# heyblackC/DFMIR

Hardware: AMD Instinct MI355X
Metric: train-step image-pairs/sec (fwd+bwd): 2D 256x256 bs=16 and 3D 160^3 bs=1 (higher is better)
Workload: dtype f32 (fp16x2-split MFMA, fp32 accumulate)

## Files before the change

dfmir_amd/_lib.py:

```python
import ctypes
import os
from ctypes import c_float, c_int, c_longlong, c_void_p, POINTER, Structure

_HERE = os.path.dirname(os.path.abspath(__file__))
LIB_PATH = os.environ.get("DFMIR_HIP_LIB") or os.path.join(_HERE, "libdfmir_hip.so")


class DfConvGeom(Structure):
    _fields_ = [(n, c_int) for n in (
        "N", "Cin", "Cout", "Di", "Hi", "Wi", "Do", "Ho", "Wo", "KD", "KH", "KW",
        "stride", "dil", "pd", "ph", "pw", "pad_mode", "act")] + [("slope", c_float)]


P = c_void_p
_GP = POINTER(DfConvGeom)
_SIGS = {
    "dfmir_abi_version": [],
    "dfmir_set_option": [ctypes.c_char_p, ctypes.c_char_p],
    "dfmir_get_option": [ctypes.c_char_p, ctypes.c_char_p, c_int],
    "dfmir_conv_fwd": [_GP, P, P, P, P, P],
    "dfmir_conv_wgrad": [_GP, P, P, P, P],
    "dfmir_bias_grad": [P, P, c_int, c_int, c_longlong, P],
    "dfmir_weight_pack": [P, P, c_int, c_int, c_int, c_int, P],
    "dfmir_weight_pack_floats": [c_int, c_int, c_int],
# ... 93 lines not shown
    "dfmir_patch_gather_bwd_amax": [P, P, P, c_int, c_int, c_longlong, c_int, P, P],
    "dfmir_patch_gather_fwd_g": [P, P, P, c_int, c_int, c_longlong, c_int, c_int, P],
    "dfmir_patch_gather_bwd_g": [P, P, P, c_int, c_int, c_longlong, c_int, c_int, P, P],
    "dfmir_l2norm_fwd": [P, P, P, c_int, c_longlong, c_float, P],
    "dfmir_l2norm_bwd": [P, P, P, P, c_int, c_longlong, c_float, P],
    "dfmir_patchnce_fwd": [P, P, P, P, c_longlong, c_int, c_int, c_float, P],
    "dfmir_patchnce_bwd": [P, P, P, P, c_longlong, c_int, c_int, c_float, P],
    "dfmir_masked_l1_fwd": [P, P, P, c_float, P, P, c_longlong, P],
    "dfmir_masked_l1_bwd": [P, P, P, c_float, P, P, P, P, c_longlong, P],
    "dfmir_flow_smooth_ws_floats": [],
    "dfmir_flow_smooth_fwd": [P, P, P] + [c_int] * 5 + [P],
    "dfmir_flow_smooth_bwd": [P, P, P] + [c_int] * 5 + [P],
    "dfmir_flow_smooth_fwd_p": [P, P, P] + [c_int] * 6 + [P],
    "dfmir_flow_smooth_bwd_p": [P, P, P] + [c_int] * 6 + [P],
    "dfmir_mul": [P, P, P, c_longlong, P],
    "dfmir_nmi_ws_floats": [c_longlong, c_int],
    "dfmir_nmi_fwd": [P, P, P, P, c_int, c_float, c_float, c_longlong, P, P, P],
    "dfmir_nmi_bwd": [P, P, P, P, c_int, c_float, c_float, c_longlong, P, P, P, P, P],
    "dfmir_warp_dice_ws_floats": [c_int] * 6,
    "dfmir_warp_dice_fwd": [c_int, P, P, P, P] + [c_int] * 6 + [P, P, P, P, P],
    "dfmir_warp_dice_bwd": [c_int, P, P, P, P] + [c_int] * 5 + [P, P, P, P],
    "dfmir_dice_ws_floats": [c_longlong, c_longlong],
    "dfmir_dice_fwd": [P, P, c_longlong, c_longlong, P, P, P],
    "dfmir_dice_bwd": [P, P, c_longlong, c_longlong, P, P, P, P, P],
    "dfmir_mse_ws_floats": [c_longlong],
    "dfmir_mse_fwd": [P, P, c_longlong, P, P, P],
    "dfmir_mse_bwd": [P, P, c_longlong, P, P, P, P],
    "dfmir_ncc_fwd_m": [P, P, P, c_int, P, P, P, P] + [c_int] * 5 + [c_float, P],
    "dfmir_ncc_bwd_m": [P, P, P, c_int, P, P, P, P, P, P] + [c_int] * 5 + [c_float, P],
    "dfmir_ncc_fwd": [P, P, P, P, P, P] + [c_int] * 5 + [c_float, P],
    "dfmir_ncc_bwd": [P, P, P, P, P, P, P, P] + [c_int] * 5 + [c_float, P],
    "dfmir_patch_gather_fwd_multi": [P, c_int, P, P, c_int, c_int, c_longlong, c_int, P],
    "dfmir_nce_head_fwd": [P, c_int, P, P, P, P, P, P, P, P, P, P, c_int, c_int, c_longlong, c_int, c_float, P],
    "dfmir_patch_ids_draw": [P, P, c_int, c_int, c_int, P, P],
    "dfmir_segment_means_fwd": [P, P, c_int, c_int, c_longlong, c_float, P],
    "dfmir_segment_means_bwd": [P, P, c_int, c_int, c_longlong, c_float, P],
    "dfmir_scalar_combine_fwd": [P, c_int, P, c_int, P, P],
    "dfmir_scalar_combine_bwd": [P, c_int, P, c_int, P, P],
    "dfmir_det_head_floats": [],
    "dfmir_det_begin": [P, c_longlong, P, c_longlong, P, c_int, P, c_longlong, P, c_int, ctypes.c_double, P],
    "dfmir_det_end": [P, P, c_longlong, P, c_longlong, P],
    "dfmir_fill_zero": [P, c_longlong, P],
    "dfmir_sum_scaled": [P, P, c_longlong, c_float, P],
    "dfmir_fill_from_scalar": [P, P, c_longlong, c_float, P],
    "dfmir_adam_step": [P, P, P, P, c_longlong] + [c_float] * 7 + [P],
}

_lib = None


class DfmirHipError(RuntimeError):
    pass


def lib():
    global _lib
    if _lib is None:
        import torch
        if not os.path.exists(LIB_PATH):
            raise DfmirHipError(
                "libdfmir_hip.so not found at %s -- build it with `python -c 'import __graft_entry__ as g; "
                "g.build()'` or `make -C dfmir_amd/csrc` (there is no CPU fallback)" % LIB_PATH)
        h = ctypes.CDLL(LIB_PATH)
        for name, args in _SIGS.items():
            fn = getattr(h, name)
            fn.argtypes = args
# ... 38 lines not shown
```

dfmir_amd/csrc/nce_head.hip:

```cpp
#include "common.h"

#define DF_IDS_MAXP 1024
#define DF_IDS_MAXPERM 4096
struct DfIdSizes {
  long long S[8];
};

__device__ __forceinline__ unsigned long long df_mix64(unsigned long long z) {
  z += 0x9E3779B97F4A7C15ull;
  z = (z ^ (z >> 30)) * 0xBF58476D1CE4E5B9ull;
  z = (z ^ (z >> 27)) * 0x94D049BB133111EBull;
  return z ^ (z >> 31);
}

__global__ __launch_bounds__(256) void patch_ids_draw_k(unsigned long long* __restrict__ state, DfIdSizes sizes,
                                                        int n_layers, int n_sets, int P, int Ppad,
                                                        long long* __restrict__ out) {
  __shared__ unsigned long long el[DF_IDS_MAXPERM];
  __shared__ unsigned char lost[DF_IDS_MAXP];
  __shared__ int pending;
  const int layer = blockIdx.x / n_sets, set = blockIdx.x - layer * n_sets;
  const unsigned long long S = (unsigned long long)sizes.S[layer];
  const unsigned long long seed = state[0], counter = state[1];
  const unsigned long long stream = df_mix64(seed ^ df_mix64(counter * 0x100000001B3ull + (unsigned long long)blockIdx.x));
// ... 253 lines not shown
  __syncthreads();
  const float nr = sqrtf((red[0][l31] + red[1][l31]) + (red[2][l31] + red[3][l31]));
  const float inv = 1.f / (nr + k.eps);
  const long long rr = r0 + l31;
  if (rr < k.rows) {
    if (k.nrm && wid == 0 && hi == 0) k.nrm[rr] = nr;
#pragma unroll
    for (int i = 0; i < 2; ++i)
#pragma unroll
      for (int e = 0; e < 16; ++e) {
        const int m = m0 + 32 * i + (e >> 2) * 8 + hi * 4 + (e & 3);
        k.out[(long long)m * k.rows + rr] = acc[i][e] * inv;
        if (k.ypre) k.ypre[(long long)m * k.rows + rr] = acc[i][e];
      }
  }
}
extern "C" int dfmir_nce_head_fwd(const float* const* srcs, int G, const long long* ids, const float* w1, const float* b1,
                                  const float* w2, const float* b2, float* out, float* nrm, float* xs, float* hs,
                                  float* ypre, int Bper, int C, long long S, int P, float eps, void* stream) {
  DF_ARG_CHECK(srcs && ids && w1 && b1 && w2 && b2 && out && G > 0 && G <= 8 && Bper > 0 && C > 0 && C <= NH_CMAX && S > 0 && P > 0);
  NceHeadP k{};
  for (int g = 0; g < G; ++g) {
    DF_ARG_CHECK(srcs[g] != nullptr);
    k.srcs.p[g] = srcs[g];
  }
  k.ids = ids; k.w1 = w1; k.b1 = b1; k.w2 = w2; k.b2 = b2;
  k.out = out; k.nrm = nrm; k.xs = xs; k.hs = hs; k.ypre = ypre;
  k.G = G; k.Bper = Bper; k.C = C; k.P = P; k.S = S; k.rows = (long long)G * Bper * P; k.eps = eps;
  nce_head_fwd_k<<<(unsigned)((k.rows + NH_R - 1) / NH_R), 256, 0, (hipStream_t)stream>>>(k);
  DF_LAUNCH_CHECK();
  return 0;
}

__global__ __launch_bounds__(256) void segment_means_k(const float* __restrict__ rows, float* __restrict__ out, int L,
                                                       int T, long long seg, float scale) {
  __shared__ float sm[17];
  const int t = blockIdx.x;
  float s = 0.f;
  for (int l = 0; l < L; ++l) {
    const float* r = rows + ((long long)l * T + t) * seg;
    for (long long i = threadIdx.x; i < seg; i += 256) s += r[i];
  }
  s = block_sum(s, sm);
  if (threadIdx.x == 0) out[t] = s * (scale / (float)seg);
}
__global__ void segment_means_bwd_k(const float* __restrict__ g, float* __restrict__ drows, int L, int T, long long seg,
                                    float scale) {
  const long long total = (long long)L * T * seg;
  for (long long i = (long long)blockIdx.x * blockDim.x + threadIdx.x; i < total;
       i += (long long)gridDim.x * blockDim.x) {
    const int t = (int)((i / seg) % T);
    drows[i] = g[t] * (scale / (float)seg);
  }
}
extern "C" int dfmir_segment_means_fwd(const float* rows, float* out, int L, int T, long long seg, float scale,
                                       void* stream) {
  DF_ARG_CHECK(rows && out && L > 0 && T > 0 && seg > 0);
  segment_means_k<<<(unsigned)T, 256, 0, (hipStream_t)stream>>>(rows, out, L, T, seg, scale);
  DF_LAUNCH_CHECK();
  return 0;
}
extern "C" int dfmir_segment_means_bwd(const float* gout, float* drows, int L, int T, long long seg, float scale,
                                       void* stream) {
  DF_ARG_CHECK(gout && drows && L > 0 && T > 0 && seg > 0);
  segment_means_bwd_k<<<df_grid((long long)L * T * seg, 256, 1024), 256, 0, (hipStream_t)stream>>>(gout, drows, L, T, seg,
                                                                                                scale);
// ... 60 lines not shown
```

dfmir_amd/csrc/patchnce.hip:

```cpp
#include "common.h"

__global__ void patch_gather_fwd_k(const float* __restrict__ feat, const long long* __restrict__ ids,
                                   float* __restrict__ out, int B, int C, long long S, int P, int bpg) {
  const long long total = (long long)B * C * P;
  for (long long i = (long long)blockIdx.x * blockDim.x + threadIdx.x; i < total;
       i += (long long)gridDim.x * blockDim.x) {
    const int p = (int)(i % P);
    const long long bc = i / P;
    const long long b = bc / C, c = bc - b * C;
    out[c * ((long long)B * P) + b * P + p] = feat[bc * S + ids[(b / bpg) * P + p]];
  }
}
template <bool DISTINCT>
__global__ void patch_gather_bwd_k(const float* __restrict__ dout, const long long* __restrict__ ids,
                                   float* __restrict__ dfeat, int B, int C, long long S, int P, int bpg,
                                   unsigned* __restrict__ amax, unsigned* __restrict__ pmax = nullptr) {
  const long long total = (long long)B * C * P;
  for (long long i = (long long)blockIdx.x * blockDim.x + threadIdx.x; i < total;
       i += (long long)gridDim.x * blockDim.x) {
    int p;
    long long bc, b, c;
    if (total < 0x7FFFFFFFLL) {
      const unsigned u = (unsigned)i;
      p = (int)(u % (unsigned)P);
      const unsigned ubc = u / (unsigned)P;
      bc = ubc; b = ubc / (unsigned)C; c = ubc - (unsigned)b * (unsigned)C;
    } else {
      p = (int)(i % P);
      bc = i / P;
      b = bc / C; c = bc - b * C;
    }
    const float v = dout[c * ((long long)B * P) + b * P + p];
    float* dst = &dfeat[bc * S + ids[(b / bpg) * P + p]];
    float old;
    if (DISTINCT) { old = *dst; *dst = old + v; }
    else old = atomicAdd(dst, v);
    if (amax) {
      float nv = fabsf(old + v);
      if (!(nv == nv)) nv = __uint_as_float(0x7f800000u);
      unsigned* sl = amax + (bc & (DF_PROBE_SLOTS - 1));
      if (__float_as_uint(nv) > *reinterpret_cast<volatile unsigned*>(sl)) atomicMax(sl, __float_as_uint(nv));
      if (pmax && __float_as_uint(nv) > *reinterpret_cast<volatile unsigned*>(pmax + bc)) atomicMax(pmax + bc, __float_as_uint(nv));
    }
  }
}

__global__ __launch_bounds__(256) void l2norm_fwd_k(const float* __restrict__ x, float* __restrict__ y,
                                                    float* __restrict__ nrm, int C, long long P, float eps) {
  __shared__ float red[16][17];
  const int r = threadIdx.x & 15, cg = threadIdx.x >> 4;
  const long long i = (long long)blockIdx.x * 16 + r;
  const bool ok = i < P;
  float s = 0.f;
  if (ok)
    for (int c = cg; c < C; c += 16) {
      const float v = x[(long long)c * P + i];
      s += v * v;
    }
  red[cg][r] = s;
  __syncthreads();
  float tot = 0.f;
#pragma unroll
  for (int g = 0; g < 16; ++g) tot += red[g][r];
  if (!ok) return;
  const float n = sqrtf(tot);
  if (cg == 0) nrm[i] = n;
  const float inv = 1.f / (n + eps);
  for (int c = cg; c < C; c += 16) y[(long long)c * P + i] = x[(long long)c * P + i] * inv;
}
__global__ __launch_bounds__(256) void l2norm_bwd_k(const float* __restrict__ dy, const float* __restrict__ x,
                                                    const float* __restrict__ nrm, float* __restrict__ dx, int C,
                                                    long long P, float eps) {
  __shared__ float red[16][17];
  const int r = threadIdx.x & 15, cg = threadIdx.x >> 4;
  const long long i = (long long)blockIdx.x * 16 + r;
  const bool ok = i < P;
  float s = 0.f;
  if (ok)
    for (int c = cg; c < C; c += 16) s += dy[(long long)c * P + i] * x[(long long)c * P + i];
// ... 286 lines not shown
  const long long r = r0 + l15;
  const float dpos = (probs[r * ld] - 1.f) * dloss[r] * invT;
#pragma unroll
  for (int t = 0; t < 4; ++t) {
    const int ct = wid * 4 + t;
    if (ct >= ntile) continue;
#pragma unroll
    for (int e = 0; e < 4; ++e) {
      const long long off = (long long)(ct * 16 + lk * 4 + e) * rows + r;
      dq[off] = acc[t][e] + dpos * k[off];
    }
  }
}

extern "C" int dfmir_patch_gather_fwd(const float* feat, const long long* ids, float* out, int B, int C,
                                      long long S, int P, void* stream) {
  DF_ARG_CHECK(feat && ids && out && B > 0 && C > 0 && S > 0 && P > 0);
  patch_gather_fwd_k<<<df_grid((long long)B * C * P, 256, 4096), 256, 0, (hipStream_t)stream>>>(
      feat, ids, out, B, C, S, P, B);
  DF_LAUNCH_CHECK();
  return 0;
}
extern "C" int dfmir_patch_gather_fwd_g(const float* feat, const long long* ids, float* out, int B, int C,
                                        long long S, int P, int G, void* stream) {
  DF_ARG_CHECK(feat && ids && out && B > 0 && C > 0 && S > 0 && P > 0 && G > 0 && B % G == 0);
  patch_gather_fwd_k<<<df_grid((long long)B * C * P, 256, 4096), 256, 0, (hipStream_t)stream>>>(
      feat, ids, out, B, C, S, P, B / G);
  DF_LAUNCH_CHECK();
  return 0;
}
extern "C" int dfmir_patch_gather_bwd_g(const float* dout, const long long* ids, float* dfeat, int B, int C,
                                        long long S, int P, int G, float* dfeat_amax, void* stream) {
  DF_ARG_CHECK(dout && ids && dfeat && B > 0 && C > 0 && S > 0 && P > 0 && G > 0 && B % G == 0);
  patch_gather_bwd_k<true><<<df_grid((long long)B * C * P, 256, 4096), 256, 0, (hipStream_t)stream>>>(
      dout, ids, dfeat, B, C, S, P, B / G, reinterpret_cast<unsigned*>(dfeat_amax));
  DF_LAUNCH_CHECK();
  return 0;
}
extern "C" int dfmir_patch_gather_bwd_gp(const float* dout, const long long* ids, float* dfeat, int B, int C,
                                         long long S, int P, int G, float* dfeat_amax, float* dfeat_pmax, void* stream) {
  DF_ARG_CHECK(dout && ids && dfeat && dfeat_amax && dfeat_pmax && B > 0 && C > 0 && S > 0 && P > 0 && G > 0 && B % G == 0);
  patch_gather_bwd_k<true><<<df_grid((long long)B * C * P, 256, 4096), 256, 0, (hipStream_t)stream>>>(
      dout, ids, dfeat, B, C, S, P, B / G, reinterpret_cast<unsigned*>(dfeat_amax), reinterpret_cast<unsigned*>(dfeat_pmax));
  DF_LAUNCH_CHECK();
  return 0;
}
extern "C" int dfmir_patch_gather_bwd_any(const float* dout, const long long* ids, float* dfeat, int B, int C,
                                          long long S, int P, int G, float* dfeat_amax, float* dfeat_pmax, void* stream) {
  DF_ARG_CHECK(dout && ids && dfeat && B > 0 && C > 0 && S > 0 && P > 0 && G > 0 && B % G == 0);
  DF_ARG_CHECK(dfeat_amax || !dfeat_pmax);
  patch_gather_bwd_k<false><<<df_grid((long long)B * C * P, 256, 4096), 256, 0, (hipStream_t)stream>>>(
      dout, ids, dfeat, B, C, S, P, B / G, reinterpret_cast<unsigned*>(dfeat_amax), reinterpret_cast<unsigned*>(dfeat_pmax));
  DF_LAUNCH_CHECK();
  return 0;
}
extern "C" int dfmir_patch_gather_bwd(const float* dout, const long long* ids, float* dfeat, int B, int C,
                                      long long S, int P, void* stream) {
  DF_ARG_CHECK(dout && ids && dfeat && B > 0 && C > 0 && S > 0 && P > 0);
  patch_gather_bwd_k<false><<<df_grid((long long)B * C * P, 256, 4096), 256, 0, (hipStream_t)stream>>>(
      dout, ids, dfeat, B, C, S, P, B, nullptr);
  DF_LAUNCH_CHECK();
  return 0;
}
extern "C" int dfmir_patch_gather_bwd_amax(const float* dout, const long long* ids, float* dfeat, int B, int C,
                                           long long S, int P, float* dfeat_amax, void* stream) {
  DF_ARG_CHECK(dout && ids && dfeat && dfeat_amax && B > 0 && C > 0 && S > 0 && P > 0);
  patch_gather_bwd_k<true><<<df_grid((long long)B * C * P, 256, 4096), 256, 0, (hipStream_t)stream>>>(
      dout, ids, dfeat, B, C, S, P, B, reinterpret_cast<unsigned*>(dfeat_amax));
  DF_LAUNCH_CHECK();
  return 0;
}
extern "C" int dfmir_l2norm_fwd(const float* x, float* y, float* norm, int C, long long rows, float eps,
                                void* stream) {
  DF_ARG_CHECK(x && y && norm && C > 0 && rows > 0);
  l2norm_fwd_k<<<(unsigned)((rows + 15) / 16), 256, 0, (hipStream_t)stream>>>(x, y, norm, C, rows, eps);
  DF_LAUNCH_CHECK();
  return 0;
}
extern "C" int dfmir_l2norm_bwd(const float* dy, const float* x, const float* norm, float* dx, int C,
                                long long rows, float eps, void* stream) {
  DF_ARG_CHECK(dy && x && norm && dx && C > 0 && rows > 0);
  l2norm_bwd_k<<<(unsigned)((rows + 15) / 16), 256, 0, (hipStream_t)stream>>>(dy, x, norm, dx, C, rows, eps);
  DF_LAUNCH_CHECK();
  return 0;
}
extern "C" int dfmir_patchnce_fwd(const float* q, const float* k, float* loss, float* probs, long long rows,
                                  int C, int G, float T, void* stream) {
  DF_ARG_CHECK(q && k && loss && probs && rows > 0 && C > 0 && G > 0 && T > 0.f);
  DF_ARG_CHECK(rows % G == 0);
  const int R = (int)(rows / G);
  DF_ARG_CHECK(R % NCE_TI == 0);
  if (R == 256 && C <= 256 && (C & 31) == 0) {
    patchnce_fwd_mfma_k<<<(unsigned)(rows / NCE_TI), 256, 0, (hipStream_t)stream>>>(q, k, loss, probs, rows, C, 1.f / T);
    DF_LAUNCH_CHECK();
    return 0;
  }
  const size_t sh = ((size_t)C * NCE_TI + 32 + 3 * NCE_TI) * sizeof(float);
  DF_ARG_CHECK(sh <= 64 * 1024);
  patchnce_fwd_k<<<(unsigned)(rows / NCE_TI), 256, sh, (hipStream_t)stream>>>(q, k, loss, probs, rows, C, R,
                                                                         1.f / T);
  DF_LAUNCH_CHECK();
// ... 21 lines not shown
```

dfmir_amd/ops.py:

```python
import ctypes
import os

import torch
from torch.autograd import Function
from torch.autograd.function import once_differentiable

from ._lib import DfConvGeom, DfmirHipError, check, lib

_VP = ctypes.c_void_p


def _p(t):
    return None if t is None else _VP(t.data_ptr())


def _st():
    return _VP(torch.cuda.current_stream().cuda_stream)


def _need(*ts):
    for t in ts:
        if t is None:
            continue
        if not t.is_cuda:
# ... 1859 lines not shown
def draw_patch_ids(sizes, n_sets, P, device):
    device = _cuda_device(device)
    st = _IDS_STATE.get(device)
    if st is None:
        st = seed_patch_ids(torch.initial_seed(), device)
    L = len(sizes)
    out = torch.empty((L, n_sets, P), device=device, dtype=torch.int64)
    sz = (ctypes.c_longlong * L)(*[int(s) for s in sizes])
    check(lib().dfmir_patch_ids_draw(_p(st), sz, L, int(n_sets), int(P), _p(out), _st()))
    return mark_distinct(out)


def patch_gather_multi(srcs, ids):
    _need(*srcs)
    _need(ids)
    G = len(srcs)
    srcs = [_c(s) for s in srcs]
    Bper, C = srcs[0].shape[0], srcs[0].shape[1]
    S = srcs[0].numel() // (Bper * C)
    for s_ in srcs:
        if tuple(s_.shape) != tuple(srcs[0].shape):
            raise DfmirHipError("patch_gather_multi: sources differ in shape")
    ids = _c(ids.to(torch.int64))
    if ids.dim() != 2 or ids.shape[0] != G:
        raise DfmirHipError("patch_gather_multi: ids must be [G, P]")
    Pn = ids.shape[1]
    out = torch.empty((C, G * Bper * Pn), device=srcs[0].device, dtype=torch.float32)
    ptrs = (ctypes.c_void_p * G)(*[s_.data_ptr() for s_ in srcs])
    check(lib().dfmir_patch_gather_fwd_multi(ptrs, G, _p(ids), _p(out), Bper, C, S, Pn, _st()))
    return out


_NO_NCE_FUSED = _env_on("DFMIR_NO_NCE_FUSED")


def nce_head_ok(C, nc, use_mlp):
    return use_mlp and not _NO_NCE_FUSED and nc == 256 and 1 <= C <= 256


def _nce_head_launch(ptrs, G, ids, mlp0, mlp2, Bper, C, S, Pn, eps, device, save):
    rows = G * Bper * Pn
    out = torch.empty((256, rows), device=device, dtype=torch.float32)
    nrm = xs = hs = ypre = None
    if save:
        nrm = torch.empty(rows, device=device, dtype=torch.float32)
        xs = torch.empty((C, rows), device=device, dtype=torch.float32)
        hs = torch.empty((256, rows), device=device, dtype=torch.float32)
        ypre = torch.empty((256, rows), device=device, dtype=torch.float32)
    arr = (ctypes.c_void_p * G)(*ptrs)
    check(lib().dfmir_nce_head_fwd(arr, G, _p(ids), _p(mlp0.packed(0)), _p(mlp0.bias), _p(mlp2.packed(0)), _p(mlp2.bias),
                                   _p(out), _p(nrm), _p(xs), _p(hs), _p(ypre), Bper, C, S, Pn, float(eps), _st()))
    return out, nrm, xs, hs, ypre


def nce_head_multi(srcs, ids, mlp0, mlp2, eps=1e-7):
    _need(*srcs)
    srcs = [_c(s_) for s_ in srcs]
    Bper, C = srcs[0].shape[0], srcs[0].shape[1]
    S = srcs[0].numel() // (Bper * C)
    ids = _c(ids.to(torch.int64))
    out, _, _, _, _ = _nce_head_launch([s_.data_ptr() for s_ in srcs], len(srcs), ids, mlp0, mlp2, Bper, C, S, ids.shape[1], eps,
                                       srcs[0].device, False)
    return out


class NceHeadFn(Function):

    @staticmethod
    def forward(ctx, feat, ids, w1, b1, w2, b2, mlp0, mlp2, eps, distinct):
        _need(feat, ids)
        ctx.stash = getattr(feat, "_df_tap_stash", None) if feat.is_contiguous() else None
        feat = _c(feat)
        ids = _c(ids.to(torch.int64))
        G, Pn = ids.shape
        B, C = feat.shape[0], feat.shape[1]
        if B % G:
            raise DfmirHipError("nce_head: ids [G,P] with G dividing the batch")
        Bper = B // G
        S = feat.numel() // (B * C)
        base = feat.data_ptr()
        ptrs = [base + 4 * g * Bper * C * S for g in range(G)]
        out, nrm, xs, hs, ypre = _nce_head_launch(ptrs, G, ids, mlp0, mlp2, Bper, C, S, Pn, eps, feat.device, True)
        ctx.save_for_backward(ids, nrm, xs, hs, ypre, w1, w2)
        ctx.meta = (tuple(feat.shape), B, C, S, Pn, G, bool(distinct), float(eps))
        ctx.mods = (mlp0, mlp2)
        return out

    @staticmethod
    @once_differentiable
    def backward(ctx, dout):
        ids, nrm, xs, hs, ypre, w1, w2 = ctx.saved_tensors
        shape, B, C, S, Pn, G, distinct, eps = ctx.meta
        mlp0, mlp2 = ctx.mods
        rows = B * Pn
        dout = _c(dout)
        dy = torch.empty_like(ypre)
        check(lib().dfmir_l2norm_bwd(_p(dout), _p(ypre), _p(nrm), _p(dy), 256, rows, eps, _st()))
        c2 = _Ctx()
        c2.cfg, c2.x_amax, c2.dead_tail, c2.in_act, c2.has_bias = (2, (1, 1, 1), 1, (0, 0, 0), 0, 0, 0.0, mlp2), None, 0, None, True
        c2.needs_input_grad = (True, ctx.needs_input_grad[4], ctx.needs_input_grad[5])
        dh, dw2, db2 = _conv_backward_impl(c2, dy.view(1, 256, 1, rows), None, hs.view(1, 256, 1, 1, rows),
                                           w2.view(256, 256, 1, 1), None)
        c1 = _Ctx()
        c1.cfg, c1.x_amax, c1.dead_tail, c1.in_act, c1.has_bias = (2, (1, 1, 1), 1, (0, 0, 0), 0, 1, 0.0, mlp0), None, 0, None, True
        c1.needs_input_grad = (ctx.needs_input_grad[0], ctx.needs_input_grad[2], ctx.needs_input_grad[3])
        dx, dw1, db1 = _conv_backward_impl(c1, dh, None, xs.view(1, C, 1, 1, rows), w1.view(256, C, 1, 1),
                                           hs.view(1, 256, 1, 1, rows))
        dfeat = None
        if dx is not None:
            dxr = _c(dx).view(C, rows)
            meta = (shape, B, C, S, Pn, G, distinct)
            if ctx.stash is not None:
                ctx.stash.append((dxr, ids, meta))
            else:
                dfeat = zeros(shape, dxr.device)
                if distinct:
                    check(lib().dfmir_patch_gather_bwd_g(_p(dxr), _p(ids), _p(dfeat), B, C, S, Pn, G, None, _st()))
                else:
                    check(lib().dfmir_patch_gather_bwd_any(_p(dxr), _p(ids), _p(dfeat), B, C, S, Pn, G, None, None, _st()))
        dw1 = dw1.view(256, C) if dw1 is not None else None
        dw2 = dw2.view(256, 256) if dw2 is not None else None
        return dfeat, None, dw1, db1, dw2, db2, None, None, None, None


def nce_head(feat, ids, mlp0, mlp2, eps=1e-7):
    groups = ids.shape[0] if ids.dim() == 2 else 1
    ids2 = ids if ids.dim() == 2 else ids.view(1, -1)
    distinct = ids_distinct(ids, groups) if (torch.is_grad_enabled() and feat.requires_grad) else True
    return NceHeadFn.apply(feat, ids2, mlp0.weight, mlp0.bias, mlp2.weight, mlp2.bias, mlp0, mlp2, eps, distinct)


_LAST_L1_WS = [None]


class MaskedL1Fn(Function):
    @staticmethod
    def forward(ctx, a, b, mask, thr):
        _need(a, b, mask)
        a, b = _c(a), _c(b)
        m = None
# ... 441 lines not shown
```

include/dfmir_hip.h:

```cpp
#ifndef DFMIR_HIP_H
#define DFMIR_HIP_H

#ifdef __cplusplus
extern "C" {
#endif

#define DFMIR_ABI_VERSION 14

int dfmir_abi_version(void);
const char* dfmir_last_error(void);

int dfmir_set_option(const char* name, const char* value);
int dfmir_get_option(const char* name, char* buf, int buf_len);

typedef struct DfConvGeom {
  int N, Cin, Cout;
  int Di, Hi, Wi;
  int Do, Ho, Wo;
  int KD, KH, KW;
  int stride, dil;
  int pd, ph, pw;
  int pad_mode;
  int act;
  float slope;
// ... 169 lines not shown
                     float* dflow, int B, int C, int D, int H, int W, int add_identity,
                     int flow_into_src, void* stream);
long long dfmir_warp_bwd_own_ws_floats(int nd, int B, int C, int D, int H, int W);
int dfmir_warp_bwd_own(int nd, const float* dout, const float* src, const float* flow, float* dsrc, float* dflow, int B,
                       int C, int D, int H, int W, int add_identity, int flow_into_src, float* ws, void* stream);

int dfmir_resize_fwd(const float* x, float* y, int planes, int Di, int Hi, int Wi, int Do, int Ho,
                     int Wo, float mult, void* stream);
int dfmir_resize_bwd(const float* dy, float* dx, int planes, int Di, int Hi, int Wi, int Do, int Ho,
                     int Wo, float mult, void* stream);
long long dfmir_resize_bwd_ws_floats(int planes, int Di, int Hi, int Wi, int Do, int Ho, int Wo);
int dfmir_resize_bwd_sep(const float* dy, float* dx, int planes, int Di, int Hi, int Wi, int Do, int Ho, int Wo,
                         float mult, float* ws, void* stream);

int dfmir_patch_gather_fwd(const float* feat, const long long* ids, float* out, int B, int C,
                           long long S, int P, void* stream);
int dfmir_patch_gather_bwd(const float* dout, const long long* ids, float* dfeat, int B, int C,
                           long long S, int P, void* stream);
int dfmir_patch_gather_bwd_amax(const float* dout, const long long* ids, float* dfeat, int B, int C, long long S,
                                int P, float* dfeat_amax, void* stream);
int dfmir_patch_gather_fwd_g(const float* feat, const long long* ids, float* out, int B, int C, long long S, int P,
                             int G, void* stream);
int dfmir_patch_gather_bwd_g(const float* dout, const long long* ids, float* dfeat, int B, int C, long long S, int P,
                             int G, float* dfeat_amax, void* stream);
int dfmir_patch_gather_bwd_gp(const float* dout, const long long* ids, float* dfeat, int B, int C, long long S, int P,
                              int G, float* dfeat_amax, float* dfeat_pmax, void* stream);
int dfmir_patch_gather_bwd_any(const float* dout, const long long* ids, float* dfeat, int B, int C, long long S, int P,
                               int G, float* dfeat_amax, float* dfeat_pmax, void* stream);
int dfmir_patch_gather_fwd_multi(const float* const* srcs, int G, const long long* ids, float* out, int Bper, int C,
                                 long long S, int P, void* stream);
int dfmir_nce_head_fwd(const float* const* srcs, int G, const long long* ids, const float* w1, const float* b1,
                       const float* w2, const float* b2, float* out, float* nrm, float* xs, float* hs, float* ypre,
                       int Bper, int C, long long S, int P, float eps, void* stream);
int dfmir_patch_ids_draw(unsigned long long* state, const long long* sizes, int n_layers, int n_sets, int P,
                         long long* out, void* stream);
int dfmir_l2norm_fwd(const float* x, float* y, float* norm, int C, long long rows, float eps, void* stream);
int dfmir_l2norm_bwd(const float* dy, const float* x, const float* norm, float* dx, int C,
                     long long rows, float eps, void* stream);
int dfmir_patchnce_fwd(const float* q, const float* k, float* loss, float* probs, long long rows,
                       int C, int G, float T, void* stream);
int dfmir_patchnce_bwd(const float* dloss, const float* probs, const float* k, float* dq,
                       long long rows, int C, int G, float T, void* stream);

int dfmir_masked_l1_fwd(const float* a, const float* b, const unsigned char* mask, float thr,
                        float* ws, float* out, long long n, void* stream);
int dfmir_masked_l1_bwd(const float* a, const float* b, const unsigned char* mask, float thr,
                        const float* ws, const float* gout, float* da, float* db, long long n,
                        void* stream);
long long dfmir_flow_smooth_ws_floats(void);
int dfmir_flow_smooth_fwd(const float* flow, float* ws, float* out, int B, int C, int D, int H,
                          int W, void* stream);
int dfmir_flow_smooth_bwd(const float* flow, const float* gout, float* dflow, int B, int C, int D,
                          int H, int W, void* stream);
int dfmir_flow_smooth_fwd_p(const float* flow, float* ws, float* out, int B, int C, int D, int H,
                            int W, int penalty, void* stream);
int dfmir_flow_smooth_bwd_p(const float* flow, const float* gout, float* dflow, int B, int C, int D,
                            int H, int W, int penalty, void* stream);
long long dfmir_nmi_ws_floats(long long n, int nb);
int dfmir_nmi_fwd(const float* y_true, const float* y_pred, const float* mask, const float* centers, int nb,
                  float preterm, float max_clip, long long n, float* ws, float* out, void* stream);
int dfmir_nmi_bwd(const float* y_true, const float* y_pred, const float* mask, const float* centers, int nb,
                  float preterm, float max_clip, long long n, const float* ws, const float* gout, float* d_true,
                  float* d_pred, void* stream);
long long dfmir_warp_dice_ws_floats(int nd, int B, int K, int D, int H, int W);
int dfmir_warp_dice_fwd(int nd, const unsigned char* mov, const unsigned char* fix, const float* flow,
                        const unsigned char* slot_of, int K, int B, int D, int H, int W, int mode, float* ws,
// ... 46 lines not shown
```

Measured before the change: 216.2.

## Fuse PatchNCE MLP head backward into data and weight-gradient kernels

Replaces the generic path for the PatchNCE projection-head backward (l2norm backward plus two 1x1 conv backwards) with two dedicated kernels. One fuses the l2norm backward, the w2 data-gradient GEMM, the ReLU mask and the w1 data-gradient GEMM per row tile using MFMA. The other computes both weight and bias gradients in a single launch with atomics. It also adds a wave-cooperative patch-gather backward scatter that reduces the amax/pmax atomics to one per wave per group. The new path uses plain fp32 MFMA instead of the split path and atomic accumulation, so summation order and numerics can differ; the old path stays behind an env flag and deterministic mode.

```diff
diff --git a/dfmir_amd/_lib.py b/dfmir_amd/_lib.py
--- a/dfmir_amd/_lib.py
+++ b/dfmir_amd/_lib.py
@@ -149,6 +149,8 @@
     "dfmir_ncc_bwd": [P, P, P, P, P, P, P, P] + [c_int] * 5 + [c_float, P],
     "dfmir_patch_gather_fwd_multi": [P, c_int, P, P, c_int, c_int, c_longlong, c_int, P],
     "dfmir_nce_head_fwd": [P, c_int, P, P, P, P, P, P, P, P, P, P, c_int, c_int, c_longlong, c_int, c_float, P],
+    "dfmir_nce_head_bwd_data": [P, P, P, P, P, P, P, P, P, c_int, c_longlong, c_float, P],
+    "dfmir_nce_head_bwd_wgrad": [P, P, P, P, P, P, P, P, c_int, c_longlong, P],
     "dfmir_patch_ids_draw": [P, P, c_int, c_int, c_int, P, P],
     "dfmir_segment_means_fwd": [P, P, c_int, c_int, c_longlong, c_float, P],
     "dfmir_segment_means_bwd": [P, P, c_int, c_int, c_longlong, c_float, P],
diff --git a/dfmir_amd/csrc/nce_head.hip b/dfmir_amd/csrc/nce_head.hip
--- a/dfmir_amd/csrc/nce_head.hip
+++ b/dfmir_amd/csrc/nce_head.hip
@@ -309,6 +309,243 @@
   return 0;
 }
 
+struct NceHeadBwdP {
+  const float *dout, *ypre, *nrm, *hs, *w1, *w2;
+  float *dy, *dh, *dx;
+  int C;
+  long long rows;
+  float eps;
+};
+__global__ __launch_bounds__(256, 2) void nce_head_bwd_data_k(NceHeadBwdP k) {
+  __shared__ float DYs[NH_M * NH_R];
+  __shared__ float DHs[NH_M * NH_R];
+  __shared__ float red[8][NH_R];
+  const int tid = threadIdx.x, lane = tid & 63, wid = tid >> 6;
+  const int l31 = lane & 31, hi = lane >> 5;
+  const long long r0 = (long long)blockIdx.x * NH_R;
+  {
+    const int r = tid & 31, cg = tid >> 5;
+    const long long rr = r0 + r;
+    const bool rok = rr < k.rows;
+    float s = 0.f;
+#pragma unroll 8
+    for (int m = cg; m < NH_M; m += 8) {
+      const float g = rok ? k.dout[(long long)m * k.rows + rr] : 0.f;
+      const float y = rok ? k.ypre[(long long)m * k.rows + rr] : 0.f;
+      DYs[m * NH_R + r] = g;
+      DHs[m * NH_R + r] = y;
+      s += g * y;
+    }
+    red[cg][r] = s;
+    __syncthreads();
+    float dot = 0.f;
+#pragma unroll
+    for (int g = 0; g < 8; ++g) dot += red[g][r];
+    const float n = rok ? k.nrm[rr] : 0.f;
+    const float inv = 1.f / (n + k.eps);
+    const float k2 = n > 0.f ? dot * inv * inv / n : 0.f;
+#pragma unroll 8
+    for (int m = cg; m < NH_M; m += 8) {
+      const float v = DYs[m * NH_R + r] * inv - DHs[m * NH_R + r] * k2;
+      DYs[m * NH_R + r] = v;
+      if (rok) k.dy[(long long)m * k.rows + rr] = v;
+    }
+  }
+  __syncthreads();
+  const int m0 = 64 * wid;
+  const long long rr = r0 + l31;
+  const bool rok = rr < k.rows;
+  nh_f32x16 acc[2];
+#pragma unroll
+  for (int i = 0; i < 2; ++i)
+#pragma unroll
+    for (int e = 0; e < 16; ++e) acc[i][e] = 0.f;
+#define NHB_GEMM(W_, LD_, MB_, SRC_)                                                              \
+  {                                                                                               \
+    const bool ok0 = m0 + l31 < (MB_), ok1 = m0 + l31 + 32 < (MB_);                               \
+    const float* wp = (W_) + m0 + l31;                                                            \
+    constexpr int nb = NH_M / 2 / NH_KB;                                                          \
+    float ca0[NH_KB], ca1[NH_KB], na0[NH_KB], na1[NH_KB];                                         \
+    _Pragma("unroll") for (int u = 0; u < NH_KB; ++u) {                                           \
+      const int kr = 2 * u + hi;                                                                  \
+      ca0[u] = ok0 ? wp[(long long)kr * (LD_)] : 0.f;                                             \
+      ca1[u] = ok1 ? wp[(long long)kr * (LD_) + 32] : 0.f;                                        \
+    }                                                                                             \
+    for (int j = 0; j < nb; ++j) {                                                                \
+      if (j + 1 < nb) {                                                                           \
+        _Pragma("unroll") for (int u = 0; u < NH_KB; ++u) {                                       \
+          const int kr = 2 * ((j + 1) * NH_KB + u) + hi;                                          \
+          na0[u] = ok0 ? wp[(long long)kr * (LD_)] : 0.f;                                         \
+          na1[u] = ok1 ? wp[(long long)kr * (LD_) + 32] : 0.f;                                    \
+        }                                                                                         \
+      }                                                                                           \
+      _Pragma("unroll") for (int u = 0; u < NH_KB; ++u) {                                         \
+        const int kr = 2 * (j * NH_KB + u) + hi;                                                  \
+        const float bv = (SRC_)[kr * NH_R + l31];                                                 \
+        acc[0] = __builtin_amdgcn_mfma_f32_32x32x2f32(ca0[u], bv, acc[0], 0, 0, 0);               \
+        acc[1] = __builtin_amdgcn_mfma_f32_32x32x2f32(ca1[u], bv, acc[1], 0, 0, 0);               \
+      }                                                                                           \
+      _Pragma("unroll") for (int u = 0; u < NH_KB; ++u) { ca0[u] = na0[u]; ca1[u] = na1[u]; }     \
+    }                                                                                             \
+  }
+  float hv[2][16];
+#pragma unroll
+  for (int i = 0; i < 2; ++i)
+#pragma unroll
+    for (int e = 0; e < 16; ++e) {
+      const int m = m0 + 32 * i + (e >> 2) * 8 + hi * 4 + (e & 3);
+      hv[i][e] = rok ? k.hs[(long long)m * k.rows + rr] : 0.f;
+    }
+  NHB_GEMM(k.w2, NH_M, NH_M, DYs)
+#pragma unroll
+  for (int i = 0; i < 2; ++i)
+#pragma unroll
+    for (int e = 0; e < 16; ++e) {
+      const int m = m0 + 32 * i + (e >> 2) * 8 + hi * 4 + (e & 3);
+      const float v = hv[i][e] > 0.f ? acc[i][e] : acc[i][e] * 0.f;
+      DHs[m * NH_R + l31] = v;
+      if (rok) k.dh[(long long)m * k.rows + rr] = v;
+      acc[i][e] = 0.f;
+    }
+  if (!k.dx) return;
+  __syncthreads();
+  if (m0 >= k.C) return;
+  NHB_GEMM(k.w1, k.C, k.C, DHs)
+#undef NHB_GEMM
+  if (rok) {
+#pragma unroll
+    for (int i = 0; i < 2; ++i)
+#pragma unroll
+      for (int e = 0; e < 16; ++e) {
+        const int c = m0 + 32 * i + (e >> 2) * 8 + hi * 4 + (e & 3);
+        if (c < k.C) k.dx[(long long)c * k.rows + rr] = acc[i][e];
+      }
+  }
+}
+extern "C" int dfmir_nce_head_bwd_data(const float* dout, const float* ypre, const float* nrm, const float* hs,
+                                       const float* w1, const float* w2, float* dy, float* dh, float* dx, int C,
+                                       long long rows, float eps, void* stream) {
+  DF_ARG_CHECK(dout && ypre && nrm && hs && w2 && dy && dh && (w1 || !dx) && C > 0 && C <= NH_CMAX && rows > 0 &&
+               rows < (1LL << 31) * NH_R);
+  NceHeadBwdP k{};
+  k.dout = dout; k.ypre = ypre; k.nrm = nrm; k.hs = hs; k.w1 = w1; k.w2 = w2;
+  k.dy = dy; k.dh = dh; k.dx = dx; k.C = C; k.rows = rows; k.eps = eps;
+  nce_head_bwd_data_k<<<(unsigned)((rows + NH_R - 1) / NH_R), 256, 0, (hipStream_t)stream>>>(k);
+  DF_LAUNCH_CHECK();
+  return 0;
+}
+
+struct NceHeadWgP {
+  const float *xs, *hs, *dy, *dh;
+  float *dw1, *db1, *dw2, *db2;
+  int C, nt2;
+  long long rows, chunks, cpb;
+};
+__global__ __launch_bounds__(256) void nce_head_bwd_wgrad_k(NceHeadWgP k) {
+  constexpr int BK = 64, LD = BK + 1;
+  __shared__ float Xs[64 * LD];
+  __shared__ float Ds[64 * LD];
+  const int tid = threadIdx.x, lane = tid & 63, wid = tid >> 6;
+  const int l31 = lane & 31, lhi = lane >> 5, wm = wid >> 1, wn = wid & 1;
+  int t = blockIdx.y;
+  const bool second = t < k.nt2;
+  if (!second) t -= k.nt2;
+  const float* x = second ? k.hs : k.xs;
+  const float* d = second ? k.dy : k.dh;
+  float* dw = second ? k.dw2 : k.dw1;
+  float* db = (t >> 2) == 0 ? (second ? k.db2 : k.db1) : nullptr;
+  const int Cin = second ? NH_M : k.C;
+  const int ci0 = (t >> 2) * 64, co0 = (t & 3) * 64;
+  const long long S = k.rows;
+  const long long cbeg = (long long)blockIdx.x * k.cpb;
+  long long cend = cbeg + k.cpb;
+  if (cend > k.chunks) cend = k.chunks;
+  if (cbeg >= cend) return;
+  const int r = tid >> 2, q16 = (tid & 3) * 16;
+  const bool xrow = dw && ci0 + r < Cin, vec = (S & 3) == 0;
+  const float* xp = x + (long long)(ci0 + r) * S;
+  const float* dp = d + (long long)(co0 + r) * S;
+  float4 rx[4], rd[4];
+  const float4 z4 = make_float4(0.f, 0.f, 0.f, 0.f);
+  float bsum = 0.f;
+  auto quad = [&](const float* p, long long q) {
+    if (vec) return q < S ? *reinterpret_cast<const float4*>(p + q) : z4;
+    return make_float4(q < S ? p[q] : 0.f, q + 1 < S ? p[q + 1] : 0.f, q + 2 < S ? p[q + 2] : 0.f,
+                       q + 3 < S ? p[q + 3] : 0.f);
+  };
+#define NW_GLOAD(c_)                                                                                         \
+  {                                                                                                          \
+    const long long q0_ = (c_) * BK + q16;                                                                   \
+    _Pragma("unroll") for (int j = 0; j < 4; ++j) {                                                          \
+      rx[j] = xrow ? quad(xp, q0_ + 4 * j) : z4;                                                             \
+      rd[j] = quad(dp, q0_ + 4 * j);                                                                         \
+    }                                                                                                        \
+  }
+#define NW_LSTORE()                                                                                          \
+  {                                                                                                          \
+    float* xs_ = &Xs[r * LD + q16];                                                                          \
+    float* ds_ = &Ds[r * LD + q16];                                                                          \
+    _Pragma("unroll") for (int j = 0; j < 4; ++j) {                                                          \
+      xs_[4 * j] = rx[j].x; xs_[4 * j + 1] = rx[j].y; xs_[4 * j + 2] = rx[j].z; xs_[4 * j + 3] = rx[j].w;    \
+      ds_[4 * j] = rd[j].x; ds_[4 * j + 1] = rd[j].y; ds_[4 * j + 2] = rd[j].z; ds_[4 * j + 3] = rd[j].w;    \
+      bsum += (rd[j].x + rd[j].y) + (rd[j].z + rd[j].w);                                                     \
+    }                                                                                                        \
+  }
+  nh_f32x16 acc;
+#pragma unroll
+  for (int i = 0; i < 16; ++i) acc[i] = 0.f;
+  NW_GLOAD(cbeg)
+  for (long long c = cbeg; c < cend; ++c) {
+    __syncthreads();
+    NW_LSTORE()
+    __syncthreads();
+    if (c + 1 < cend) NW_GLOAD(c + 1)
+    if (dw) {
+      const float* ap = &Xs[(wm * 32 + l31) * LD + lhi];
+      const float* bp = &Ds[(wn * 32 + l31) * LD + lhi];
+#pragma unroll 8
+      for (int ks = 0; ks < BK / 2; ++ks)
+        acc = __builtin_amdgcn_mfma_f32_32x32x2f32(ap[2 * ks], bp[2 * ks], acc, 0, 0, 0);
+    }
+  }
+#undef NW_GLOAD
+#undef NW_LSTORE
+  if (dw) {
+    const int co = co0 + wn * 32 + l31;
+#pragma unroll
+    for (int i = 0; i < 16; ++i) {
+      const int ci = ci0 + wm * 32 + 4 * lhi + (i & 3) + 8 * (i >> 2);
+      if (ci < Cin) atomicAdd(dw + (long long)ci * NH_M + co, acc[i]);
+    }
+  }
+  bsum += __shfl_xor(bsum, 1);
+  bsum += __shfl_xor(bsum, 2);
+  if (db && (tid & 3) == 0) atomicAdd(db + co0 + r, bsum);
+}
+extern "C" int dfmir_nce_head_bwd_wgrad(const float* xs, const float* hs, const float* dy, const float* dh, float* dw1,
+                                        float* db1, float* dw2, float* db2, int C, long long rows, void* stream) {
+  DF_ARG_CHECK(xs && hs && dy && dh && (dw1 || db1 || dw2 || db2) && C > 0 && C <= NH_CMAX && rows > 0);
+  DF_ARG_CHECK(((reinterpret_cast<uintptr_t>(xs) | reinterpret_cast<uintptr_t>(hs) | reinterpret_cast<uintptr_t>(dy) |
+                 reinterpret_cast<uintptr_t>(dh)) & 15) == 0);
+  NceHeadWgP k{};
+  k.xs = xs; k.hs = hs; k.dy = dy; k.dh = dh; k.dw1 = dw1; k.db1 = db1; k.dw2 = dw2; k.db2 = db2;
+  k.C = C; k.rows = rows;
+  k.nt2 = dw2 ? 4 * (NH_M / 64) : (db2 ? 4 : 0);
+  const int nt1 = dw1 ? 4 * ((C + 63) / 64) : (db1 ? 4 : 0);
+  const int nt = k.nt2 + nt1;
+  k.chunks = (rows + 63) / 64;
+  long long want = 1024 / nt;
+  long long maxs = (k.chunks + 7) / 8;
+  if (want > maxs) want = maxs;
+  if (want < 1) want = 1;
+  k.cpb = (k.chunks + want - 1) / want;
+  const unsigned nx = (unsigned)((k.chunks + k.cpb - 1) / k.cpb);
+  DF_ARG_CHECK(nx <= 65535u);
+  nce_head_bwd_wgrad_k<<<dim3(nx, (unsigned)nt), 256, 0, (hipStream_t)stream>>>(k);
+  DF_LAUNCH_CHECK();
+  return 0;
+}
+
 __global__ __launch_bounds__(256) void segment_means_k(const float* __restrict__ rows, float* __restrict__ out, int L,
                                                        int T, long long seg, float scale) {
   __shared__ float sm[17];
diff --git a/dfmir_amd/csrc/patchnce.hip b/dfmir_amd/csrc/patchnce.hip
--- a/dfmir_amd/csrc/patchnce.hip
+++ b/dfmir_amd/csrc/patchnce.hip
@@ -45,6 +45,65 @@
   }
 }
 
+__global__ __launch_bounds__(256) void patch_gather_bwd_wave_k(const float* __restrict__ dout,
+                                                               const long long* __restrict__ ids,
+                                                               float* __restrict__ dfeat, int B, int C, long long S, int P,
+                                                               int bpg, unsigned* __restrict__ amax,
+                                                               unsigned* __restrict__ pmax) {
+  const long long total = (long long)B * C * P;
+  const int lane = threadIdx.x & 63;
+  for (long long base = (long long)blockIdx.x * blockDim.x + (threadIdx.x & ~63); base < total;
+       base += (long long)gridDim.x * blockDim.x) {
+    const long long i = base + lane;
+    const bool live = i < total;
+    long long bc = -1;
+    unsigned nvb = 0u;
+    if (live) {
+      int p;
+      long long b, c;
+      if (total < 0x7FFFFFFFLL) {
+        const unsigned u = (unsigned)i;
+        p = (int)(u % (unsigned)P);
+        const unsigned ubc = u / (unsigned)P;
+        bc = ubc; b = ubc / (unsigned)C; c = ubc - (unsigned)b * (unsigned)C;
+      } else {
+        p = (int)(i % P);
+        bc = i / P;
+        b = bc / C; c = bc - b * C;
+      }
+      const float v = dout[c * ((long long)B * P) + b * P + p];
+      float* dst = &dfeat[bc * S + ids[(b / bpg) * P + p]];
+      const float old = *dst;
+      *dst = old + v;
+      float nv = fabsf(old + v);
+      if (!(nv == nv)) nv = __uint_as_float(0x7f800000u);
+      nvb = __float_as_uint(nv);
+    }
+    unsigned long long todo = __ballot(live);
+    while (todo) {
+      const int lead = __ffsll((long long)todo) - 1;
+      const long long lbc = __shfl(bc, lead);
+      const bool mine = live && bc == lbc;
+      unsigned m = mine ? nvb : 0u;
+#pragma unroll
+      for (int o = 32; o > 0; o >>= 1) {
+        const unsigned t = (unsigned)__shfl_xor((int)m, o);
+        m = t > m ? t : m;
+      }
+      if (lane == lead) {
+        unsigned* sl = amax + (lbc & (DF_PROBE_SLOTS - 1));
+        if (m > *reinterpret_cast<volatile unsigned*>(sl)) atomicMax(sl, m);
+        if (pmax && m > *reinterpret_cast<volatile unsigned*>(pmax + lbc)) atomicMax(pmax + lbc, m);
+      }
+      todo &= ~__ballot(mine);
+    }
+  }
+}
+static bool df_scatter_per_element() {
+  static DfOptFlag o{"DFMIR_NO_NCE_BWD_FUSED"};
+  return o.get();
+}
+
 __global__ __launch_bounds__(256) void l2norm_fwd_k(const float* __restrict__ x, float* __restrict__ y,
                                                     float* __restrict__ nrm, int C, long long P, float eps) {
   __shared__ float red[16][17];
@@ -397,16 +456,24 @@
 extern "C" int dfmir_patch_gather_bwd_g(const float* dout, const long long* ids, float* dfeat, int B, int C,
                                         long long S, int P, int G, float* dfeat_amax, void* stream) {
   DF_ARG_CHECK(dout && ids && dfeat && B > 0 && C > 0 && S > 0 && P > 0 && G > 0 && B % G == 0);
-  patch_gather_bwd_k<true><<<df_grid((long long)B * C * P, 256, 4096), 256, 0, (hipStream_t)stream>>>(
-      dout, ids, dfeat, B, C, S, P, B / G, reinterpret_cast<unsigned*>(dfeat_amax));
+  if (dfeat_amax && !df_scatter_per_element())
+    patch_gather_bwd_wave_k<<<df_grid((long long)B * C * P, 256, 4096), 256, 0, (hipStream_t)stream>>>(
+        dout, ids, dfeat, B, C, S, P, B / G, reinterpret_cast<unsigned*>(dfeat_amax), nullptr);
+  else
+    patch_gather_bwd_k<true><<<df_grid((long long)B * C * P, 256, 4096), 256, 0, (hipStream_t)stream>>>(
+        dout, ids, dfeat, B, C, S, P, B / G, reinterpret_cast<unsigned*>(dfeat_amax));
   DF_LAUNCH_CHECK();
   return 0;
 }
 extern "C" int dfmir_patch_gather_bwd_gp(const float* dout, const long long* ids, float* dfeat, int B, int C,
                                          long long S, int P, int G, float* dfeat_amax, float* dfeat_pmax, void* stream) {
   DF_ARG_CHECK(dout && ids && dfeat && dfeat_amax && dfeat_pmax && B > 0 && C > 0 && S > 0 && P > 0 && G > 0 && B % G == 0);
-  patch_gather_bwd_k<true><<<df_grid((long long)B * C * P, 256, 4096), 256, 0, (hipStream_t)stream>>>(
-      dout, ids, dfeat, B, C, S, P, B / G, reinterpret_cast<unsigned*>(dfeat_amax), reinterpret_cast<unsigned*>(dfeat_pmax));
+  if (!df_scatter_per_element())
+    patch_gather_bwd_wave_k<<<df_grid((long long)B * C * P, 256, 4096), 256, 0, (hipStream_t)stream>>>(
+        dout, ids, dfeat, B, C, S, P, B / G, reinterpret_cast<unsigned*>(dfeat_amax), reinterpret_cast<unsigned*>(dfeat_pmax));
+  else
+    patch_gather_bwd_k<true><<<df_grid((long long)B * C * P, 256, 4096), 256, 0, (hipStream_t)stream>>>(
+        dout, ids, dfeat, B, C, S, P, B / G, reinterpret_cast<unsigned*>(dfeat_amax), reinterpret_cast<unsigned*>(dfeat_pmax));
   DF_LAUNCH_CHECK();
   return 0;
 }
@@ -430,8 +497,12 @@
 extern "C" int dfmir_patch_gather_bwd_amax(const float* dout, const long long* ids, float* dfeat, int B, int C,
                                            long long S, int P, float* dfeat_amax, void* stream) {
   DF_ARG_CHECK(dout && ids && dfeat && dfeat_amax && B > 0 && C > 0 && S > 0 && P > 0);
-  patch_gather_bwd_k<true><<<df_grid((long long)B * C * P, 256, 4096), 256, 0, (hipStream_t)stream>>>(
-      dout, ids, dfeat, B, C, S, P, B, reinterpret_cast<unsigned*>(dfeat_amax));
+  if (!df_scatter_per_element())
+    patch_gather_bwd_wave_k<<<df_grid((long long)B * C * P, 256, 4096), 256, 0, (hipStream_t)stream>>>(
+        dout, ids, dfeat, B, C, S, P, B, reinterpret_cast<unsigned*>(dfeat_amax), nullptr);
+  else
+    patch_gather_bwd_k<true><<<df_grid((long long)B * C * P, 256, 4096), 256, 0, (hipStream_t)stream>>>(
+        dout, ids, dfeat, B, C, S, P, B, reinterpret_cast<unsigned*>(dfeat_amax));
   DF_LAUNCH_CHECK();
   return 0;
 }
diff --git a/dfmir_amd/ops.py b/dfmir_amd/ops.py
--- a/dfmir_amd/ops.py
+++ b/dfmir_amd/ops.py
@@ -1915,6 +1915,7 @@
 
 
 _NO_NCE_FUSED = _env_on("DFMIR_NO_NCE_FUSED")
+_NO_NCE_BWD_FUSED = _env_on("DFMIR_NO_NCE_BWD_FUSED")
 
 
 def nce_head_ok(C, nc, use_mlp):
@@ -1945,6 +1946,27 @@
     out, _, _, _, _ = _nce_head_launch([s_.data_ptr() for s_ in srcs], len(srcs), ids, mlp0, mlp2, Bper, C, S, ids.shape[1], eps,
                                        srcs[0].device, False)
     return out
+
+
+def _nce_lin_targets(owner, weight, need_w, need_b):
+    Cout, Cin = weight.shape[0], weight.shape[1]
+    defer = (_DEFER["on"] and getattr(owner, "weight", None) is not None and owner.weight.grad is not None
+             and owner.weight.grad.is_contiguous())
+    dw = db = None
+    fresh_w = fresh_b = False
+    if need_b:
+        bias = getattr(owner, "bias", None)
+        bg = bias.grad if (defer and bias is not None) else None
+        if bg is not None and bg.is_contiguous():
+            db = bg
+        else:
+            db, fresh_b = zeros(Cout, weight.device), True
+    if need_w:
+        if defer:
+            dw = _deferred_buffer(owner, 1, Cin, Cout, (Cout, Cin, 1, 1), weight.device)
+        else:
+            dw, fresh_w = zeros((1, Cin, Cout), weight.device), True
+    return dw, db, fresh_w, fresh_b
 
 
 class NceHeadFn(Function):
@@ -1978,17 +2000,32 @@
         rows = B * Pn
         dout = _c(dout)
         dy = torch.empty_like(ypre)
-        check(lib().dfmir_l2norm_bwd(_p(dout), _p(ypre), _p(nrm), _p(dy), 256, rows, eps, _st()))
-        c2 = _Ctx()
-        c2.cfg, c2.x_amax, c2.dead_tail, c2.in_act, c2.has_bias = (2, (1, 1, 1), 1, (0, 0, 0), 0, 0, 0.0, mlp2), None, 0, None, True
-        c2.needs_input_grad = (True, ctx.needs_input_grad[4], ctx.needs_input_grad[5])
-        dh, dw2, db2 = _conv_backward_impl(c2, dy.view(1, 256, 1, rows), None, hs.view(1, 256, 1, 1, rows),
-                                           w2.view(256, 256, 1, 1), None)
-        c1 = _Ctx()
-        c1.cfg, c1.x_amax, c1.dead_tail, c1.in_act, c1.has_bias = (2, (1, 1, 1), 1, (0, 0, 0), 0, 1, 0.0, mlp0), None, 0, None, True
-        c1.needs_input_grad = (ctx.needs_input_grad[0], ctx.needs_input_grad[2], ctx.needs_input_grad[3])
-        dx, dw1, db1 = _conv_backward_impl(c1, dh, None, xs.view(1, C, 1, 1, rows), w1.view(256, C, 1, 1),
-                                           hs.view(1, 256, 1, 1, rows))
+        if _NO_NCE_BWD_FUSED or _DET["on"]:
+            check(lib().dfmir_l2norm_bwd(_p(dout), _p(ypre), _p(nrm), _p(dy), 256, rows, eps, _st()))
+            c2 = _Ctx()
+            c2.cfg, c2.x_amax, c2.dead_tail, c2.in_act, c2.has_bias = (2, (1, 1, 1), 1, (0, 0, 0), 0, 0, 0.0, mlp2), None, 0, None, True
+            c2.needs_input_grad = (True, ctx.needs_input_grad[4], ctx.needs_input_grad[5])
+            dh, dw2, db2 = _conv_backward_impl(c2, dy.view(1, 256, 1, rows), None, hs.view(1, 256, 1, 1, rows),
+                                               w2.view(256, 256, 1, 1), None)
+            c1 = _Ctx()
+            c1.cfg, c1.x_amax, c1.dead_tail, c1.in_act, c1.has_bias = (2, (1, 1, 1), 1, (0, 0, 0), 0, 1, 0.0, mlp0), None, 0, None, True
+            c1.needs_input_grad = (ctx.needs_input_grad[0], ctx.needs_input_grad[2], ctx.needs_input_grad[3])
+            dx, dw1, db1 = _conv_backward_impl(c1, dh, None, xs.view(1, C, 1, 1, rows), w1.view(256, C, 1, 1),
+                                               hs.view(1, 256, 1, 1, rows))
+        else:
+            w1c, w2c = _c(w1), _c(w2)
+            dh = torch.empty_like(hs)
+            dx = torch.empty_like(xs) if ctx.needs_input_grad[0] else None
+            check(lib().dfmir_nce_head_bwd_data(_p(dout), _p(ypre), _p(nrm), _p(hs), _p(w1c), _p(w2c), _p(dy), _p(dh), _p(dx),
+                                                C, rows, eps, _st()))
+            t1 = _nce_lin_targets(mlp0, w1, ctx.needs_input_grad[2], ctx.needs_input_grad[3])
+            t2 = _nce_lin_targets(mlp2, w2, ctx.needs_input_grad[4], ctx.needs_input_grad[5])
+            if any(t_ is not None for t_ in t1[:2] + t2[:2]):
+                check(lib().dfmir_nce_head_bwd_wgrad(_p(xs), _p(hs), _p(dy), _p(dh), _p(t1[0]), _p(t1[1]), _p(t2[0]), _p(t2[1]),
+                                                     C, rows, _st()))
+            dw1 = weight_unpack(t1[0], (256, C, 1, 1)) if t1[2] else None
+            dw2 = weight_unpack(t2[0], (256, 256, 1, 1)) if t2[2] else None
+            db1, db2 = (t1[1] if t1[3] else None), (t2[1] if t2[3] else None)
         dfeat = None
         if dx is not None:
             dxr = _c(dx).view(C, rows)
diff --git a/include/dfmir_hip.h b/include/dfmir_hip.h
--- a/include/dfmir_hip.h
+++ b/include/dfmir_hip.h
@@ -225,6 +225,11 @@
 int dfmir_nce_head_fwd(const float* const* srcs, int G, const long long* ids, const float* w1, const float* b1,
                        const float* w2, const float* b2, float* out, float* nrm, float* xs, float* hs, float* ypre,
                        int Bper, int C, long long S, int P, float eps, void* stream);
+int dfmir_nce_head_bwd_data(const float* dout, const float* ypre, const float* nrm, const float* hs, const float* w1,
+                            const float* w2, float* dy, float* dh, float* dx, int C, long long rows, float eps,
+                            void* stream);
+int dfmir_nce_head_bwd_wgrad(const float* xs, const float* hs, const float* dy, const float* dh, float* dw1, float* db1,
+                             float* dw2, float* db2, int C, long long rows, void* stream);
 int dfmir_patch_ids_draw(unsigned long long* state, const long long* sizes, int n_layers, int n_sets, int P,
                          long long* out, void* stream);
 int dfmir_l2norm_fwd(const float* x, float* y, float* norm, int C, long long rows, float eps, void* stream);
```

Measured after the change: 215.6. Within noise of the previous version (-0.3%).
